# bitlayer-org/tap-stark

Measured on AMD Instinct MI355X. Metric: trace cells/sec (proofs/sec alongside), 2^20x64 BabyBear trace, higher is better.
Workload: dtype u32

## Files before the change

tap-stark_amd/csrc/ntt_lde.hip:

```cpp
#include <stdlib.h>

#include <optional>
#include <type_traits>

#include "ntt_rounds.hpp"

namespace ts {

template <int LM, bool SKIP_R16 = false>
__global__ void __launch_bounds__(chunk_threads(LM))
k_intt_contig(uint32_t* __restrict__ data, uint64_t col_stride, unsigned log_n,
              const uint32_t* __restrict__ Winv, uint32_t* __restrict__ data2, uint32_t gw) {
    __shared__ uint32_t s[padded(1 << LM)];
    const uint32_t c = blockIdx.x;
    uint32_t* col = blockIdx.y < gw ? data + (uint64_t)blockIdx.y * col_stride
                                    : data2 + (uint64_t)(blockIdx.y - gw) * col_stride;
    uint32_t* g = col + ((uint64_t)c << LM);
    chunk_load<LM>(s, g);
    chunk_rounds<LM, true, SKIP_R16>(s, log_n - LM, c, Winv);
    chunk_store<LM, false>(s, g);
}

__global__ void __launch_bounds__(256)
k_transpose_bitrev_r16(const uint32_t* __restrict__ src, uint32_t* __restrict__ dst, unsigned log_n,
                       uint32_t w, uint64_t dst_col_stride, uint32_t src_width,
                       const uint32_t* __restrict__ Winv) {
    __shared__ uint32_t tile[64][65];
    const uint32_t p0 = blockIdx.x << 6;
    const uint32_t c0 = blockIdx.y * 64;
    const uint32_t tx = threadIdx.x & 63, ty = threadIdx.x >> 6;
    const uint32_t rb = bitrev32(p0, log_n);
    const uint64_t row_step = (uint64_t)src_width << (log_n - 6);
    uint32_t v[16];
    if (c0 + tx < w) {
        const uint32_t* sp = src + (uint64_t)rb * src_width + c0 + tx;
#pragma unroll
        for (int q = 0; q < 16; q++) v[q] = sp[(uint64_t)(__brev(16 * ty + (uint32_t)q) >> 26) * row_step];
    } else {
#pragma unroll
        for (int q = 0; q < 16; q++) v[q] = 0;
    }
    radix_butterflies<4, true, false>(v, log_n - 4, 0, 0, (p0 >> 4) + ty, Winv);
#pragma unroll
    for (int q = 0; q < 16; q++) tile[16 * ty + q][tx] = v[q];
    __syncthreads();
    uint32_t t[16];
#pragma unroll
    for (int k = 0; k < 16; k++) t[k] = tile[tx][ty + 4 * k];
    uint32_t* dp = dst + (uint64_t)(c0 + ty) * dst_col_stride + p0 + tx;
#pragma unroll
    for (int k = 0; k < 16; k++)
        if (c0 + ty + 4 * k < w) dp[(uint64_t)(4 * k) * dst_col_stride] = t[k];
}

template <int LM, int CPW>
__device__ __forceinline__ void lde_fwd_contig_block(uint32_t* __restrict__ out, uint64_t out_col_stride, unsigned log_n,
                                                     const uint32_t* __restrict__ W, const uint32_t beta) {
    __shared__ uint32_t s[padded(1 << LM)];
    constexpr int NT = chunk_threads(LM);
    constexpr int NV = (1 << LM) / 4 / NT;
    uint32_t* col = out + (uint64_t)blockIdx.y * out_col_stride + ((uint64_t)beta << log_n);
    if constexpr (CPW == 1) {
        const uint32_t c = blockIdx.x;
        uint32_t* o = col + ((uint64_t)c << LM);
        chunk_load<LM>(s, o);
        chunk_rounds<LM, false>(s, log_n - LM, c, W);
        chunk_store<LM, true>(s, o);
    } else {
        const uint32_t c0 = blockIdx.x * CPW;
        uint4 v[NV];
        {
            const uint4* g4 = reinterpret_cast<const uint4*>(col + ((uint64_t)c0 << LM));
#pragma unroll
            for (int k = 0; k < NV; k++) v[k] = g4[threadIdx.x + (uint32_t)k * NT];
        }
#pragma unroll 1
        for (int i = 0; i < CPW; i++) {
            const uint32_t c = c0 + i;
#pragma unroll
            for (int k = 0; k < NV; k++) {
                const uint32_t i4 = threadIdx.x + (uint32_t)k * NT;
                const uint32_t a = 4 * i4 + (i4 >> 3);
                s[a] = v[k].x;
                s[a + 1] = v[k].y;
                s[a + 2] = v[k].z;
                s[a + 3] = v[k].w;
            }
            __syncthreads();
            if (i + 1 < CPW) {
                const uint4* g4 = reinterpret_cast<const uint4*>(col + ((uint64_t)(c + 1) << LM));
#pragma unroll
                for (int k = 0; k < NV; k++) v[k] = g4[threadIdx.x + (uint32_t)k * NT];
            }
            chunk_rounds<LM, false>(s, log_n - LM, c, W);
            chunk_store<LM, true>(s, col + ((uint64_t)c << LM));
            __syncthreads();
        }
    }
}

template <int LM, int CPW = 1>
__global__ void __launch_bounds__(chunk_threads(LM), CPW > 1 ? 4 : 1)
k_lde_fwd_contig(uint32_t* __restrict__ out, uint64_t out_col_stride, unsigned log_n,
                 const uint32_t* __restrict__ W) {
    lde_fwd_contig_block<LM, CPW>(out, out_col_stride, log_n, W, blockIdx.z);
}

template <int LM, int CPW = 1>
__global__ void __launch_bounds__(chunk_threads(LM), CPW > 1 ? 4 : 1)
k_lde_fwd_contig_own(uint32_t* __restrict__ out, uint64_t out_col_stride, unsigned log_n,
                     const uint32_t* __restrict__ W, uint32_t gw, uint32_t own_a, uint32_t own_b) {
    const uint32_t own = blockIdx.y < gw ? own_a : own_b;
    lde_fwd_contig_block<LM, CPW>(out, out_col_stride, log_n, W, blockIdx.z + (blockIdx.z >= own ? 1u : 0u));
}

template <int PLAN, int TILE = TILE_ELEMS, int NTM = NT_MID, int LM = LOG_M, bool OWN = false>
__global__ void __launch_bounds__(NTM)
k_lde_mid(const uint32_t* __restrict__ evals, uint64_t in_col_stride, uint32_t* __restrict__ out,
          uint64_t out_col_stride, unsigned log_n, unsigned log_len, unsigned log_T,
          unsigned row_shift, unsigned beta0, unsigned n_cosets, const uint32_t* __restrict__ W,
          const uint32_t* __restrict__ Winv, const uint32_t* __restrict__ scale_a,
          const uint32_t* __restrict__ evals2, const uint32_t* __restrict__ scale_b, uint32_t gw,
          uint32_t own_a, uint32_t own_b) {
    __shared__ uint32_t s[padded(TILE)];
    constexpr int PER_THREAD = TILE / NTM;
    if (PLAN == 1) {
        log_len = 8;
        log_T = 5;
    }
    const bool remap = PLAN == 0 && log_T < 5 && gridDim.x >= 8;
    uint32_t bx = remap ? (blockIdx.x & 7) * (gridDim.x >> 3) + (blockIdx.x >> 3) : blockIdx.x;
    uint32_t col_id = blockIdx.y;
    if constexpr (PLAN == 1) {
        const uint32_t ncols = gridDim.x >> (LM - 5);
        bx = (blockIdx.x & 31) + 32 * (blockIdx.x / (32 * ncols));
        col_id = (blockIdx.x >> 5) % ncols;
    }
    const uint32_t j2_0 = bx << log_T;
    const uint32_t* g = (col_id < gw ? evals + (uint64_t)col_id * in_col_stride
                                     : evals2 + (uint64_t)(col_id - gw) * in_col_stride) + j2_0;
    const uint32_t* __restrict__ scale = col_id < gw ? scale_a : scale_b;
    const uint32_t own = OWN ? (col_id < gw ? own_a : own_b) : 0xffffffffu;
    const uint32_t total = 1u << (log_len + log_T);
    const uint32_t tmask = (1u << log_T) - 1;
    if constexpr (PLAN == 1) {
        uint32_t t[PER_THREAD];
#pragma unroll
        for (int k = 0; k < PER_THREAD; k++) {
            const uint32_t i = threadIdx.x + (uint32_t)k * NTM;
            t[k] = g[((uint64_t)(i >> log_T) << row_shift) + (i & tmask)];
        }
#pragma unroll
        for (int k = 0; k < PER_THREAD; k++) s[pad(threadIdx.x + (uint32_t)k * NTM)] = t[k];
    } else {
        for (uint32_t i = threadIdx.x; i < total; i += NTM)
            s[pad(i)] = g[((uint64_t)(i >> log_T) << row_shift) + (i & tmask)];
    }
    __syncthreads();
    if (PLAN == 1) {
        radix_round<4, true, 5, NTM>(s, 13, 4, 0, 0, Winv);
    } else {
        tile_inverse_rt<NTM>(s, log_len, log_T, 0, 0, Winv);
    }
    uint32_t coef[PER_THREAD];
#pragma unroll
    for (int k = 0; k < PER_THREAD; k++) {
        const uint32_t i = threadIdx.x + (uint32_t)k * NTM;
        coef[k] = i < total ? s[pad(i)] : 0u;
    }
    constexpr int GP = PER_THREAD / 16;
    if constexpr (PLAN == 1) {
#pragma unroll
        for (int j = 0; j < GP; j++) {
            uint32_t v[16];
#pragma unroll
            for (int q = 0; q < 16; q++) v[q] = coef[j + GP * q];
            radix_butterflies<4, true, true>(v, 0, 0, 0, 0, Winv);
#pragma unroll
            for (int q = 0; q < 16; q++) coef[j + GP * q] = v[q];
        }
    }
    constexpr bool PREFETCH = PLAN == 1;
    uint32_t scv[PREFETCH ? 16 : 1];
    const uint32_t* scp = nullptr;
    if constexpr (PREFETCH) {
        const uint32_t i0 = threadIdx.x;
        scp = scale + ((uint64_t)(i0 >> 5) << LM) + (i0 & 31) + j2_0;
        const uint32_t first = OWN && own == 0 ? 1u : 0u;
#pragma unroll
        for (int q = 0; q < 16; q++)
            scv[q] = (scp + ((uint64_t)(beta0 + first) << log_n))[(uint64_t)q * (NTM >> 5) << LM];
    }
    for (uint32_t bl = 0; bl < n_cosets; bl++) {
        if (OWN && bl == own) continue;
        const uint32_t beta = beta0 + bl;
        const uint32_t* sc = scale + ((uint64_t)beta << log_n);
        __syncthreads();
        if constexpr (PLAN == 1) {
#pragma unroll
            for (int j = 0; j < GP; j++) {
                uint32_t v[16];
#pragma unroll
                for (int q = 0; q < 16; q++) v[q] = mont_mul_lazy(coef[j + GP * q], scv[q]);
                const uint32_t nb = OWN && bl + 1 == own ? bl + 2 : bl + 1;
                if (nb < n_cosets) {
                    const uint32_t* nx = scp + ((uint64_t)(beta0 + nb) << log_n);
#pragma unroll
                    for (int q = 0; q < 16; q++) scv[q] = nx[(uint64_t)q * (NTM >> 5) << LM];
                }
                radix_butterflies<4, false, true>(v, 0, 0, 0, 0, W);
#pragma unroll
                for (int q = 0; q < 16; q++) s[pad(threadIdx.x + (uint32_t)(j + GP * q) * NTM)] = v[q];
            }
            __syncthreads();
            uint32_t* og = out + (uint64_t)col_id * out_col_stride + ((uint64_t)bl << log_n) + j2_0;
            radix_round<4, false, 5, NTM>(s, 13, 4, 0, 0, W);
            uint32_t t[PER_THREAD];
#pragma unroll
            for (int k = 0; k < PER_THREAD; k++) t[k] = s[pad(threadIdx.x + (uint32_t)k * NTM)];
            uint32_t* ot = og + ((uint64_t)(threadIdx.x >> 5) << LM) + (threadIdx.x & 31);
#pragma unroll
            for (int k = 0; k < PER_THREAD; k++) ot[(uint64_t)k * (NTM >> 5) << LM] = t[k];
            continue;
        } else {
#pragma unroll
            for (int k = 0; k < PER_THREAD; k++) {
                const uint32_t i = threadIdx.x + (uint32_t)k * NTM;
                if (i < total) {
                    const uint32_t kk = ((i >> log_T) << row_shift) + (i & tmask) + j2_0;
                    s[pad(i)] = mont_mul_lazy(coef[k], sc[kk]);
                }
            }
            __syncthreads();
            tile_forward_rt<NTM>(s, log_len, log_T, 0, 0, W);
        }
        uint32_t* o = out + (uint64_t)col_id * out_col_stride + ((uint64_t)bl << log_n) + j2_0;
        if (row_shift != 0) {
            for (uint32_t i = threadIdx.x; i < total; i += NTM)
                o[((uint64_t)(i >> log_T) << row_shift) + (i & tmask)] = s[pad(i)];
        } else {
            for (uint32_t i = threadIdx.x; i < total; i += NTM)
                o[((uint64_t)(i >> log_T) << row_shift) + (i & tmask)] = red2p(s[pad(i)]);
        }
    }
}

template <bool VEC>
__global__ void __launch_bounds__(256)
k_lde_own_copy(const uint32_t* __restrict__ evals, uint64_t in_col_stride, uint32_t* __restrict__ out,
               uint64_t out_col_stride, unsigned log_n, const uint32_t* __restrict__ evals2, uint32_t gw,
               uint32_t own_a, uint32_t own_b) {
    const uint32_t col = blockIdx.y;
    const uint32_t* src = col < gw ? evals + (uint64_t)col * in_col_stride
                                   : evals2 + (uint64_t)(col - gw) * in_col_stride;
    uint32_t* dst = out + (uint64_t)col * out_col_stride + ((uint64_t)(col < gw ? own_a : own_b) << log_n);
    if constexpr (VEC) {
        const uint4* s4 = reinterpret_cast<const uint4*>(src) + (uint64_t)blockIdx.x * 1024 + threadIdx.x;
        uint4* d4 = reinterpret_cast<uint4*>(dst) + (uint64_t)blockIdx.x * 1024 + threadIdx.x;
        uint4 v[4];
#pragma unroll
        for (int k = 0; k < 4; k++) v[k] = s4[256 * k];
#pragma unroll
        for (int k = 0; k < 4; k++) d4[256 * k] = v[k];
    } else {
        const uint64_t i = (uint64_t)blockIdx.x * 256 + threadIdx.x;
        if (i < (1ull << log_n)) dst[i] = src[i];
    }
}

constexpr const char* INTT_NAME[3] = {"k_intt_contig<12>", "k_intt_contig<13>", "k_intt_contig<14>"};
constexpr const char* INTT_R16_NAME[3] = {"(k_intt_contig<12, true>)", "(k_intt_contig<13, true>)",
                                          "(k_intt_contig<14, true>)"};
constexpr const char* FWD_NAME[3] = {"k_lde_fwd_contig<12>", "k_lde_fwd_contig<13>", "(k_lde_fwd_contig<14, 4>)"};

template <class F>
static void with_chunk_log(unsigned LM, F&& f) {
    if (LM == 12) f(std::integral_constant<int, 12>{});
    else if (LM == 13) f(std::integral_constant<int, 13>{});
    else f(std::integral_constant<int, 14>{});
}

bool launch_transpose_bitrev_r16(Context& ctx, const uint32_t* src, uint32_t* dst, unsigned log_n, uint32_t w,
                                 uint64_t dst_col_stride, uint32_t src_width) {
    if (w == 0 || !ntt_plan(log_n).fused_first_round) return false;
    ctx.ensure_twiddles(log_n);
    TS_LAUNCH(ctx, k_transpose_bitrev_r16, dim3(1u << (log_n - 6), (w + 63) / 64), dim3(256), 0, src, dst, log_n, w,
              dst_col_stride, src_width ? src_width : w, (const uint32_t*)ctx.d_twiddle_inv);
    TS_HIP(hipGetLastError());
    return true;
}

void launch_contig_inverse(Context& ctx, const NttPlan& p, uint32_t* data, uint64_t col_stride, uint32_t ncols,
                           bool first_round_done, uint32_t* data2, uint32_t gw) {
    const uint32_t* Winv = ctx.d_twiddle_inv;
    with_chunk_log(p.LM, [&](auto lm) {
        constexpr int LM = decltype(lm)::value;
        const dim3 g(p.chunks, ncols), b(chunk_threads(LM));
        if (first_round_done)
            TS_LAUNCH_NAMED(ctx, INTT_R16_NAME[LM - 12], (k_intt_contig<LM, true>), g, b, 0, data, col_stride, p.log_n,
                            Winv, data2, gw);
        else
            TS_LAUNCH_NAMED(ctx, INTT_NAME[LM - 12], k_intt_contig<LM>, g, b, 0, data, col_stride, p.log_n, Winv, data2,
                            gw);
    });
}

static void launch_lde_mid(Context& ctx, const NttPlan& p, const uint32_t* evals, uint64_t in_col_stride,
                           uint32_t* out, uint64_t out_col_stride, uint32_t ncols, uint32_t beta0, uint32_t n_beta,
                           const uint32_t* scale, const uint32_t* evals2, const uint32_t* scale2, uint32_t gw,
                           uint32_t own_a, uint32_t own_b) {
    const uint32_t *W = ctx.d_twiddle_fwd, *Winv = ctx.d_twiddle_inv;
    const dim3 grid(p.tiles, ncols), b(NT_MID);
    const dim3 grid1(p.tiles * ncols);
#define TS_MID_ARGS \
    evals, in_col_stride, out, out_col_stride, p.log_n, p.log_len, p.log_T, p.row_shift, beta0, n_beta, W, Winv, scale, \
        evals2, scale2, gw, own_a, own_b
    if (own_a != LDE_NO_OWN && p.mid == NttMid::FIXED256 && p.LM == 12)
        TS_LAUNCH_NAMED(ctx, "k_lde_mid<1>", (k_lde_mid<1, TILE_ELEMS, NT_MID, 12, true>), grid1, b, 0, TS_MID_ARGS);
    else if (own_a != LDE_NO_OWN && p.mid == NttMid::FIXED256 && p.LM == 13)
        TS_LAUNCH_NAMED(ctx, "(k_lde_mid<1, 8192, 512, 13>)", (k_lde_mid<1, 8192, 512, 13, true>), grid1, b, 0,
                        TS_MID_ARGS);
    else if (own_a != LDE_NO_OWN && p.mid == NttMid::FIXED256)
        TS_LAUNCH_NAMED(ctx, "(k_lde_mid<1, 8192, 512, 14>)", (k_lde_mid<1, 8192, 512, 14, true>), grid1, b, 0,
                        TS_MID_ARGS);
    else if (own_a != LDE_NO_OWN)
        TS_LAUNCH_NAMED(ctx, "k_lde_mid<0>", (k_lde_mid<0, TILE_ELEMS, NT_MID, LOG_M, true>), grid, b, 0, TS_MID_ARGS);
    else if (p.mid == NttMid::TILE16384)
        TS_LAUNCH_NAMED(ctx, "(k_lde_mid<0, 16384>)", (k_lde_mid<0, 16384>), grid, b, 0, TS_MID_ARGS);
    else if (p.mid == NttMid::FIXED256 && p.LM == 12)
        TS_LAUNCH_NAMED(ctx, "k_lde_mid<1>", k_lde_mid<1>, grid1, b, 0, TS_MID_ARGS);
    else if (p.mid == NttMid::FIXED256 && p.LM == 13)
        TS_LAUNCH_NAMED(ctx, "(k_lde_mid<1, 8192, 512, 13>)", (k_lde_mid<1, 8192, 512, 13>), grid1, b, 0, TS_MID_ARGS);
    else if (p.mid == NttMid::FIXED256)
        TS_LAUNCH_NAMED(ctx, "(k_lde_mid<1, 8192, 512, 14>)", (k_lde_mid<1, 8192, 512, 14>), grid1, b, 0, TS_MID_ARGS);
    else
        TS_LAUNCH_NAMED(ctx, "k_lde_mid<0>", k_lde_mid<0>, grid, b, 0, TS_MID_ARGS);
#undef TS_MID_ARGS
}

void launch_contig_forward(Context& ctx, const NttPlan& p, uint32_t* data, uint64_t col_stride, uint32_t ncols,
                           uint32_t n_blocks, uint32_t gw, uint32_t own_a, uint32_t own_b) {
    const uint32_t* W = ctx.d_twiddle_fwd;
    with_chunk_log(p.LM, [&](auto lm) {
        constexpr int LM = decltype(lm)::value;
        constexpr int CPW = LM == 14 ? 4 : 1;
        if (own_a != LDE_NO_OWN)
            TS_LAUNCH_NAMED(ctx, FWD_NAME[LM - 12], (k_lde_fwd_contig_own<LM, CPW>),
                            dim3(p.chunks / CPW, ncols, n_blocks - 1), dim3(chunk_threads(LM)), 0, data, col_stride,
                            p.log_n, W, gw, own_a, own_b);
        else
            TS_LAUNCH_NAMED(ctx, FWD_NAME[LM - 12], (k_lde_fwd_contig<LM, CPW>), dim3(p.chunks / CPW, ncols, n_blocks),
                            dim3(chunk_threads(LM)), 0, data, col_stride, p.log_n, W);
    });
}

int lde_own_coset_used(unsigned log_n, unsigned log_blowup, uint32_t shift) {
    if (const char* e = getenv("TS_LDE_OWN_COSET"); e && *e && atoi(e) == 0) return -1;
    if (log_blowup == 0 || log_n + log_blowup > 27 || ntt_plan(log_n).mid == NttMid::TILE16384) return -1;
    return lde_own_coset(log_n, log_blowup, shift);
}

void coset_lde(Context& ctx, uint32_t* evals, uint64_t in_col_stride, uint32_t ncols, unsigned log_n,
               unsigned log_blowup, uint32_t shift, uint32_t* out, uint64_t out_col_stride,
               uint32_t beta0, uint32_t n_beta, bool first_round_done, uint32_t* evals2, uint32_t shift2,
               uint32_t gw, bool stage_timers) {
    if (ncols == 0) return;
    TS_REQUIRE(evals2 == nullptr || (gw >= 1 && gw < ncols && shift2 != 0), TS_ERR_INVALID,
               "coset_lde: second matrix needs its first column and its shift");
    if (evals2 == nullptr) gw = 0xffffffffu;
    TS_REQUIRE(log_n + log_blowup <= 27, TS_ERR_INVALID, "coset_lde: log_n + log_blowup > 27");
    const NttPlan p = ntt_plan(log_n);
    ntt_require_shape(p, ncols, in_col_stride, out_col_stride, true);
    TS_REQUIRE(!first_round_done || p.fused_first_round, TS_ERR_INVARIANT,
               "coset_lde: no contiguous inverse pass at this size");
    ctx.ensure_twiddles(log_n == 0 ? 1 : log_n);

    const uint32_t n_cosets = 1u << log_blowup;
    if (n_beta == 0) n_beta = n_cosets - beta0;
    TS_REQUIRE(beta0 < n_cosets && n_beta <= n_cosets - beta0, TS_ERR_INVALID, "coset_lde: coset range");
    const uint32_t* scale = coset_scale_table(ctx, log_n, log_blowup, shift);
    const uint32_t* scale2 = evals2 ? coset_scale_table(ctx, log_n, log_blowup, shift2) : nullptr;

    uint32_t own_a = LDE_NO_OWN, own_b = LDE_NO_OWN;
    if (beta0 == 0 && n_beta == n_cosets && !first_round_done && ctx.lde_pass_mask == 7u) {
        const int a = lde_own_coset_used(log_n, log_blowup, shift);
        const int b = evals2 ? lde_own_coset_used(log_n, log_blowup, shift2) : a;
        if (a >= 0 && b >= 0) {
            own_a = (uint32_t)a;
            own_b = (uint32_t)b;
            const uint64_t n = 1ull << log_n;
            if (p.two_pass)
                TS_LAUNCH_NAMED(ctx, "k_lde_own_copy", k_lde_own_copy<true>, dim3((unsigned)(n >> 12), ncols), dim3(256), 0,
                                (const uint32_t*)evals, in_col_stride, out, out_col_stride, log_n,
                                (const uint32_t*)evals2, gw, own_a, own_b);
            else
                TS_LAUNCH_NAMED(ctx, "k_lde_own_copy", k_lde_own_copy<false>, dim3((unsigned)((n + 255) / 256), ncols),
                                dim3(256), 0, (const uint32_t*)evals, in_col_stride, out, out_col_stride, log_n,
                                (const uint32_t*)evals2, gw, own_a, own_b);
        }
    }

    if (!p.two_pass) {
        launch_lde_mid(ctx, p, evals, in_col_stride, out, out_col_stride, ncols, beta0, n_beta, scale, evals2, scale2,
                       gw, own_a, own_b);
    } else {
        if (ctx.lde_pass_mask & 1u) {
            std::optional<StageTimer> t;
            if (stage_timers) t.emplace(&ctx, "lde: inverse NTT, contiguous stages");
            launch_contig_inverse(ctx, p, evals, in_col_stride, ncols, first_round_done, evals2, gw);
        }
        std::optional<StageTimer> t_rest;
        if (stage_timers) t_rest.emplace(&ctx, "lde: strided pass + forward NTT of the owned cosets");
        if (ctx.lde_pass_mask & 2u)
            launch_lde_mid(ctx, p, evals, in_col_stride, out, out_col_stride, ncols, beta0, n_beta, scale, evals2,
                           scale2, gw, own_a, own_b);
        if (ctx.lde_pass_mask & 4u) launch_contig_forward(ctx, p, out, out_col_stride, ncols, n_beta, gw, own_a, own_b);
    }
    TS_HIP(hipGetLastError());
}

}
```

tap-stark_amd/csrc/open.hip:

```cpp
#include "kernels.hpp"

namespace ts {

__device__ __forceinline__ uint32_t root_bitrev(const uint32_t* __restrict__ W, unsigned L, uint64_t r) {
    if (L == 0) return R_MOD_P;
    uint32_t w = W[((uint64_t)1 << (L - 1)) + (r >> 1)];
    return (r & 1) ? neg(w) : w;
}

constexpr int BW_ROWS = 4;

__global__ void __launch_bounds__(256)
k_bary_weights(unsigned log_n, const uint32_t* __restrict__ W, uint32_t gen_mont, Ef z0, Ef z1,
               uint32_t n_points, Ef* __restrict__ out) {
    const uint64_t n = 1ull << log_n;
    const uint64_t t0 = ((uint64_t)blockIdx.x * blockDim.x + threadIdx.x) * BW_ROWS;
    if (t0 >= n) return;
    Ef num[2 * BW_ROWS];
    uint32_t nrm[2 * BW_ROWS], pre[2 * BW_ROWS], xs[BW_ROWS];
    uint32_t run = R_MOD_P;
#pragma unroll
    for (int k = 0; k < BW_ROWS; k++) {
        const bool ok = t0 + k < n;
        uint32_t x = ok ? mont_mul(gen_mont, root_bitrev(W, log_n, t0 + k)) : R_MOD_P;
        xs[k] = x;
#pragma unroll
        for (int p = 0; p < 2; p++) {
            const Ef z = p == 0 ? z0 : z1;
            Ef u = Ef{{sub(z.c[0], x), z.c[1], z.c[2], z.c[3]}};
            if (p < (int)n_points && ok) {
                ef_inv_parts(u, num[2 * k + p], nrm[2 * k + p]);
            } else {
                num[2 * k + p] = ef_zero();
                nrm[2 * k + p] = R_MOD_P;
            }
            pre[2 * k + p] = run;
            run = mont_mul(run, nrm[2 * k + p]);
        }
    }
    uint32_t inv = mont_inv(run);
#pragma unroll
    for (int j = 2 * BW_ROWS - 1; j >= 0; j--) {
        uint32_t ninv = mont_mul(inv, pre[j]);
        inv = mont_mul(inv, nrm[j]);
        const int k = j >> 1, p = j & 1;
        if (p < (int)n_points && t0 + k < n)
            out[(uint64_t)p * n + t0 + k] = ef_mul_base(num[j], mont_mul(ninv, xs[k]));
    }
}

void launch_bary_weights(Context& ctx, unsigned log_n, const Ef* points_mont, uint32_t n_points,
                         Ef* out, uint32_t coset_gen) {
    TS_REQUIRE(n_points >= 1 && n_points <= 2, TS_ERR_INVALID, "bary_weights: 1 or 2 points");
    ctx.ensure_twiddles(log_n == 0 ? 1 : log_n);
    const uint64_t threads = (((uint64_t)1 << log_n) + BW_ROWS - 1) / BW_ROWS;
    Ef z0 = points_mont[0], z1 = n_points > 1 ? points_mont[1] : points_mont[0];
    TS_LAUNCH(ctx, k_bary_weights, dim3((unsigned)((threads + 255) / 256)), dim3(256), 0, log_n,
              ctx.d_twiddle_fwd, to_mont(coset_gen ? coset_gen : GENERATOR), z0, z1, n_points, out);
    TS_HIP(hipGetLastError());
}

template <int NP, int COLS>
__global__ void __launch_bounds__(256)
k_bary_dots(const uint32_t* __restrict__ m, uint64_t col_stride, uint32_t width, unsigned log_n,
            const Ef* __restrict__ weights, uint32_t* __restrict__ partial, uint32_t rows_per_block) {
    constexpr int RS = 64 / COLS;
    constexpr int TR = 16 * 4 * RS;
    constexpr int PER_THREAD = COLS * TR / 256;
    __shared__ uint32_t tile[16 * 257];
    __shared__ uint32_t wts[TR][NP * 4];
    __shared__ uint32_t red[4 * RS][COLS][NP * 4];
    const uint64_t n = 1ull << log_n;
    const uint32_t c0 = blockIdx.y * COLS;
    const uint32_t lane = threadIdx.x & 63, wv = threadIdx.x >> 6;
    const uint32_t cl = lane % COLS, rs = lane / COLS;
    const uint32_t sub = wv * RS + rs;
    const uint64_t row_begin = (uint64_t)blockIdx.x * rows_per_block;
    const uint64_t row_end = row_begin + rows_per_block < n ? row_begin + rows_per_block : n;
    uint64_t acc[NP * 4];
#pragma unroll
    for (int j = 0; j < NP * 4; j++) acc[j] = 0;
    for (uint64_t row0 = row_begin; row0 < row_end; row0 += TR) {
        uint32_t v[PER_THREAD];
#pragma unroll
        for (int k = 0; k < PER_THREAD; k++) {
            const uint32_t e = threadIdx.x + (uint32_t)k * 256;
            const uint32_t c = c0 + e / TR;
            const uint64_t t = row0 + e % TR;
            v[k] = (c < width && t < row_end) ? m[(uint64_t)c * col_stride + t] : 0u;
        }
        for (uint32_t e = threadIdx.x; e < (uint32_t)(TR * NP); e += 256) {
            const uint32_t p = e / TR, tt = e % TR;
            const uint64_t t = row0 + tt;
            Ef w = ef_zero();
            if (t < row_end) w = weights[(uint64_t)p * n + t];
            wts[tt][p * 4 + 0] = w.c[0];
            wts[tt][p * 4 + 1] = w.c[1];
            wts[tt][p * 4 + 2] = w.c[2];
            wts[tt][p * 4 + 3] = w.c[3];
        }
#pragma unroll
        for (int k = 0; k < PER_THREAD; k++) {
            const uint32_t e = threadIdx.x + (uint32_t)k * 256;
            const uint32_t t = e % TR;
            tile[(t & 15) * 257 + (t >> 4) * COLS + e / TR] = v[k];
        }
        __syncthreads();
#pragma unroll
        for (int rr = 0; rr < 16; rr++) {
            const uint32_t tt = sub * 16 + rr;
            const uint32_t x = tile[rr * 257 + sub * COLS + cl];
#pragma unroll
            for (int j = 0; j < NP * 4; j++) acc[j] = lazy_mac(acc[j], x, wts[tt][j]);
            if (rr & 1) {
#pragma unroll
                for (int j = 0; j < NP * 4; j++) acc[j] = lazy_fix(acc[j]);
            }
        }
        __syncthreads();
    }
#pragma unroll
    for (int j = 0; j < NP * 4; j++) red[sub][cl][j] = lazy_finish(acc[j]);
    __syncthreads();
    for (uint32_t idx = threadIdx.x; idx < (uint32_t)(COLS * NP * 4); idx += 256) {
        const uint32_t c = idx / (NP * 4), j = idx % (NP * 4);
        uint32_t sum = 0;
#pragma unroll
        for (int q = 0; q < 4 * RS; q++) sum = add(sum, red[q][c][j]);
        if (c0 + c < width)
            partial[((uint64_t)blockIdx.x * width + c0 + c) * (NP * 4) + j] = sum;
    }
}

struct BaryFinishJob {
    const uint32_t* partial;
    uint32_t* out;
    uint32_t n_blocks, n_words;
};
__device__ __forceinline__ void bary_finish_group(const uint32_t* __restrict__ partial, uint32_t* __restrict__ out,
                                                  uint32_t n_blocks, uint32_t n_words, uint32_t group) {
    __shared__ uint32_t red[4][4];
    const uint32_t j = group * 4 + (threadIdx.x & 3);
    uint32_t v = 0;
    if (j < n_words) {
        uint32_t b = threadIdx.x >> 2;
        for (; b + 7 * 64 < n_blocks; b += 8 * 64) {
            uint32_t x[8];
#pragma unroll
            for (int k = 0; k < 8; k++) x[k] = partial[(uint64_t)(b + 64 * k) * n_words + j];
#pragma unroll
            for (int k = 0; k < 8; k++) v = add(v, x[k]);
        }
        for (; b < n_blocks; b += 64) v = add(v, partial[(uint64_t)b * n_words + j]);
    }
#pragma unroll
    for (int off = 32; off >= 4; off >>= 1) v = add(v, __shfl_down(v, off, 64));
    const uint32_t lane = threadIdx.x & 63, wv = threadIdx.x >> 6;
    if (lane < 4) red[wv][lane] = v;
    __syncthreads();
    if (threadIdx.x < 4 && j < n_words)
        out[j] = add(add(red[0][threadIdx.x], red[1][threadIdx.x]),
                     add(red[2][threadIdx.x], red[3][threadIdx.x]));
}
__global__ void __launch_bounds__(256)
k_bary_finish(BaryFinishJob j0, BaryFinishJob j1, uint32_t g0) {
    const bool first = blockIdx.x < g0;
    bary_finish_group(first ? j0.partial : j1.partial, first ? j0.out : j1.out, first ? j0.n_blocks : j1.n_blocks,
                      first ? j0.n_words : j1.n_words, first ? blockIdx.x : blockIdx.x - g0);
}
__global__ void __launch_bounds__(256)
k_bary_finish3(BaryFinishJob j0, BaryFinishJob j1, BaryFinishJob j2, uint32_t g0, uint32_t g1) {
    const BaryFinishJob j = blockIdx.x < g0 ? j0 : blockIdx.x < g0 + g1 ? j1 : j2;
    bary_finish_group(j.partial, j.out, j.n_blocks, j.n_words,
                      blockIdx.x < g0 ? blockIdx.x : blockIdx.x < g0 + g1 ? blockIdx.x - g0 : blockIdx.x - g0 - g1);
}

__global__ void __launch_bounds__(256)
k_bary_finish4(BaryFinishJob j0, BaryFinishJob j1, BaryFinishJob j2, BaryFinishJob j3, uint32_t g0, uint32_t g1,
               uint32_t g2) {
    const uint32_t b = blockIdx.x;
    const BaryFinishJob j = b < g0 ? j0 : b < g0 + g1 ? j1 : b < g0 + g1 + g2 ? j2 : j3;
    bary_finish_group(j.partial, j.out, j.n_blocks, j.n_words,
                      b < g0 ? b : b < g0 + g1 ? b - g0 : b < g0 + g1 + g2 ? b - g0 - g1 : b - g0 - g1 - g2);
}

void launch_bary_finish(Context& ctx, BaryPending& pend) {
    if (pend.n == 0) return;
    BaryFinishJob j[4] = {{nullptr, nullptr, 0, 0}, {nullptr, nullptr, 0, 0}, {nullptr, nullptr, 0, 0},
                          {nullptr, nullptr, 0, 0}};
    uint32_t g[4] = {0, 0, 0, 0};
    for (uint32_t i = 0; i < pend.n; i++) {
        j[i] = BaryFinishJob{pend.partial[i].p, pend.out[i], pend.n_blocks[i], pend.n_words[i]};
        g[i] = (pend.n_words[i] + 3) / 4;
    }
    if (pend.n == 4)
        TS_LAUNCH(ctx, k_bary_finish4, dim3(g[0] + g[1] + g[2] + g[3]), dim3(256), 0, j[0], j[1], j[2], j[3], g[0], g[1],
                  g[2]);
    else if (pend.n == 3)
        TS_LAUNCH(ctx, k_bary_finish3, dim3(g[0] + g[1] + g[2]), dim3(256), 0, j[0], j[1], j[2], g[0], g[1]);
    else
        TS_LAUNCH(ctx, k_bary_finish, dim3(g[0] + g[1]), dim3(256), 0, j[0], j[1], g[0]);
    TS_HIP(hipGetLastError());
    for (uint32_t i = 0; i < pend.n; i++) pend.partial[i].reset();
    pend.n = 0;
}

void launch_bary_dots(Context& ctx, const ColMat& m, unsigned log_n, const Ef* weights,
                      uint32_t n_points, Ef* out, BaryPending* pending) {
    const uint64_t n = 1ull << log_n;
    const bool narrow = m.width <= 8;
    const uint32_t tr = narrow ? 512 : 64;
    uint32_t n_blocks = (uint32_t)((n + tr - 1) / tr);
    if (n_blocks > 2048) n_blocks = 2048;
    uint32_t rows_per_block = (uint32_t)(((n + n_blocks - 1) / n_blocks + tr - 1) / tr * tr);
    n_blocks = (uint32_t)((n + rows_per_block - 1) / rows_per_block);
    const uint32_t n_words = m.width * n_points * 4;
    DevBuf<uint32_t> partial(&ctx, (size_t)n_blocks * n_words);
    const uint32_t* md = m.d;
    if (narrow) {
        dim3 grid(n_blocks, (m.width + 7) / 8);
        if (n_points == 2)
            TS_LAUNCH(ctx, (k_bary_dots<2, 8>), grid, dim3(256), 0, md, m.col_stride, m.width, log_n,
                      weights, partial.p, rows_per_block);
        else
            TS_LAUNCH(ctx, (k_bary_dots<1, 8>), grid, dim3(256), 0, md, m.col_stride, m.width, log_n,
                      weights, partial.p, rows_per_block);
    } else {
        dim3 grid(n_blocks, (m.width + 63) / 64);
        if (n_points == 2)
            TS_LAUNCH(ctx, (k_bary_dots<2, 64>), grid, dim3(256), 0, md, m.col_stride, m.width, log_n,
                      weights, partial.p, rows_per_block);
        else
            TS_LAUNCH(ctx, (k_bary_dots<1, 64>), grid, dim3(256), 0, md, m.col_stride, m.width, log_n,
                      weights, partial.p, rows_per_block);
    }
    TS_HIP(hipGetLastError());
    BaryPending own;
    BaryPending& pend = pending ? *pending : own;
    if (pend.n == pend.capacity) launch_bary_finish(ctx, pend);
    pend.partial[pend.n] = std::move(partial);
    pend.out[pend.n] = reinterpret_cast<uint32_t*>(out);
    pend.n_blocks[pend.n] = n_blocks;
    pend.n_words[pend.n] = n_words;
    pend.n++;
    if (!pending) launch_bary_finish(ctx, pend);
}

__device__ __forceinline__ void row_dot_acc(uint64_t (&acc)[4], const uint32_t* __restrict__ m,
                                            uint64_t col_stride, uint32_t width, uint64_t X,
                                            const uint32_t* __restrict__ weights) {
    uint64_t a0 = acc[0], a1 = acc[1], a2 = acc[2], a3 = acc[3];
    constexpr int B = 8;
    const uint32_t* col = m + X;
    uint32_t i = 0;
    for (; i + B <= width; i += B) {
        uint32_t v[B];
#pragma unroll
        for (int k = 0; k < B; k++) v[k] = col[(uint64_t)(i + k) * col_stride];
#pragma unroll
        for (int k = 0; k < B; k++) {
            const uint32_t* ap = weights + 4 * (i + k);
            a0 = lazy_mac(a0, v[k], ap[0]);
            a1 = lazy_mac(a1, v[k], ap[1]);
            a2 = lazy_mac(a2, v[k], ap[2]);
            a3 = lazy_mac(a3, v[k], ap[3]);
            if (k & 1) {
                a0 = lazy_fix(a0);
                a1 = lazy_fix(a1);
                a2 = lazy_fix(a2);
                a3 = lazy_fix(a3);
            }
        }
    }
    if (i < width) {
        uint32_t v[B];
#pragma unroll
        for (int k = 0; k < B; k++) v[k] = i + k < width ? col[(uint64_t)(i + k) * col_stride] : 0u;
#pragma unroll
        for (int k = 0; k < B; k++) {
            if (i + k < width) {
                const uint32_t* ap = weights + 4 * (i + k);
                a0 = lazy_mac(a0, v[k], ap[0]);
                a1 = lazy_mac(a1, v[k], ap[1]);
                a2 = lazy_mac(a2, v[k], ap[2]);
                a3 = lazy_mac(a3, v[k], ap[3]);
            }
            if (k & 1) {
                a0 = lazy_fix(a0);
                a1 = lazy_fix(a1);
                a2 = lazy_fix(a2);
                a3 = lazy_fix(a3);
            }
        }
    }
    acc[0] = a0; acc[1] = a1; acc[2] = a2; acc[3] = a3;
}
__device__ __forceinline__ Ef row_dot_alpha(const uint32_t* __restrict__ m, uint64_t col_stride,
                                            uint32_t width, uint64_t X,
                                            const uint32_t* __restrict__ alpha_pows) {
    uint64_t acc[4] = {0, 0, 0, 0};
    row_dot_acc(acc, m, col_stride, width, X, alpha_pows);
    return Ef{{lazy_finish(acc[0]), lazy_finish(acc[1]), lazy_finish(acc[2]), lazy_finish(acc[3])}};
}

template <int NP>
__device__ __forceinline__ void inv_denoms(uint32_t x_mont, const Ef* z_mont, Ef* out) {
    Ef num[NP];
    uint32_t nrm[NP];
#pragma unroll
    for (int p = 0; p < NP; p++) {
        const Ef z = z_mont[p];
        Ef u = Ef{{sub(x_mont, z.c[0]), neg(z.c[1]), neg(z.c[2]), neg(z.c[3])}};
        ef_inv_parts(u, num[p], nrm[p]);
    }
    if (NP == 2) {
        uint32_t inv = mont_inv(mont_mul(nrm[0], nrm[NP - 1]));
        out[0] = ef_mul_base(num[0], mont_mul(inv, nrm[NP - 1]));
        out[NP - 1] = ef_mul_base(num[NP - 1], mont_mul(inv, nrm[0]));
    } else {
        out[0] = ef_mul_base(num[0], mont_inv(nrm[0]));
    }
}

template <int NP>
__global__ void __launch_bounds__(256)
k_reduce(const uint32_t* __restrict__ m, uint64_t col_stride, uint32_t width, unsigned log_h,
         const uint32_t* __restrict__ W, uint32_t gen_mont, const uint32_t* __restrict__ alpha_pows,
         ReduceArgs args, Ef* __restrict__ ro) {
    const uint64_t h = 1ull << log_h;
    const uint64_t X = (uint64_t)blockIdx.x * blockDim.x + threadIdx.x;
    if (X >= h) return;
    const Ef S = row_dot_alpha(m, col_stride, width, X, alpha_pows);
    const uint32_t x = mont_mul(gen_mont, root_bitrev(W, log_h, X));
    Ef inv_d[NP];
    inv_denoms<NP>(x, args.z_mont, inv_d);
    Ef acc = args.accumulate ? ro[X] : ef_zero();
#pragma unroll
    for (int p = 0; p < NP; p++) {
        Ef t = ef_mul(ef_sub(S, args.rys[p]), args.off_mont[p]);
        acc = ef_add(acc, ef_mul(t, inv_d[p]));
    }
    ro[X] = acc;
}

void launch_reduce(Context& ctx, const ColMat& m, unsigned log_h, const uint32_t* d_alpha_pows_mont,
                   const ReduceArgs& args, Ef* ro) {
    TS_REQUIRE(args.n_points >= 1 && args.n_points <= 2, TS_ERR_INVALID, "reduce: 1 or 2 points");
    ctx.ensure_twiddles(log_h == 0 ? 1 : log_h);
    const uint64_t h = 1ull << log_h;
    dim3 grid((unsigned)((h + 255) / 256));
    if (args.n_points == 2)
        TS_LAUNCH(ctx, k_reduce<2>, grid, dim3(256), 0, (const uint32_t*)m.d, m.col_stride, m.width,
                  log_h, (const uint32_t*)ctx.d_twiddle_fwd, to_mont(GENERATOR), d_alpha_pows_mont, args,
                  ro);
    else
        TS_LAUNCH(ctx, k_reduce<1>, grid, dim3(256), 0, (const uint32_t*)m.d, m.col_stride, m.width,
                  log_h, (const uint32_t*)ctx.d_twiddle_fwd, to_mont(GENERATOR), d_alpha_pows_mont, args,
                  ro);
    TS_HIP(hipGetLastError());
}

__global__ void __launch_bounds__(256)
k_reduce_fused(const uint32_t* __restrict__ trace, uint64_t trace_stride, uint32_t width,
               unsigned log_h, const uint32_t* __restrict__ W, uint32_t gen_mont,
               const uint32_t* __restrict__ alpha_pows, FusedReduceArgs a, Ef* __restrict__ ro) {
    const uint64_t X = (uint64_t)blockIdx.x * blockDim.x + threadIdx.x;
    if (X >= a.rows) return;
    const Ef St = row_dot_alpha(trace, trace_stride, width, X, alpha_pows);
    const uint32_t x = mont_mul(gen_mont, root_bitrev(W, log_h, a.row0 + X));
    Ef inv_d[2];
    inv_denoms<2>(x, a.z_mont, inv_d);
    uint64_t acc[4] = {0, 0, 0, 0};
    uint32_t c = 0;
    for (; c + 2 <= a.n_chunks; c += 2) {
        uint32_t v[8];
#pragma unroll
        for (int k = 0; k < 8; k++) v[k] = a.chunk[c + (k >> 2)][(uint64_t)(k & 3) * a.chunk_stride + X];
        const uint32_t* ap = a.chunk_w + 16 * c;
#pragma unroll
        for (int k = 0; k < 8; k++) {
#pragma unroll
            for (int j = 0; j < 4; j++) acc[j] = lazy_mac(acc[j], v[k], ap[4 * k + j]);
            if (k & 1) {
#pragma unroll
                for (int j = 0; j < 4; j++) acc[j] = lazy_fix(acc[j]);
            }
        }
    }
    for (; c < a.n_chunks; c++) row_dot_acc(acc, a.chunk[c], a.chunk_stride, 4, X, a.chunk_w + 16 * c);
    const Ef D{{lazy_finish(acc[0]), lazy_finish(acc[1]), lazy_finish(acc[2]), lazy_finish(acc[3])}};
    const Ef g0 = ef_sub(ef_add(ef_mul(St, a.off_t[0]), D), a.k0);
    const Ef g1 = ef_sub(ef_mul(St, a.off_t[1]), a.k1);
    const Ef r = ef_add(ef_mul(g0, inv_d[0]), ef_mul(g1, inv_d[1]));
    *reinterpret_cast<uint4*>(ro + X) = make_uint4(r.c[0], r.c[1], r.c[2], r.c[3]);
}

struct PrepReduceArgs {
    const uint32_t* prep;
    uint64_t stride;
    uint32_t width;
    Ef off_p[2];
};
__global__ void __launch_bounds__(256)
k_reduce_fused_pre(const uint32_t* __restrict__ trace, uint64_t trace_stride, uint32_t width,
               unsigned log_h, const uint32_t* __restrict__ W, uint32_t gen_mont,
               const uint32_t* __restrict__ alpha_pows, FusedReduceArgs a, PrepReduceArgs pa,
               Ef* __restrict__ ro) {
    const uint64_t X = (uint64_t)blockIdx.x * blockDim.x + threadIdx.x;
    if (X >= a.rows) return;
    const Ef St = row_dot_alpha(trace, trace_stride, width, X, alpha_pows);
    const uint32_t x = mont_mul(gen_mont, root_bitrev(W, log_h, a.row0 + X));
    Ef inv_d[2];
    inv_denoms<2>(x, a.z_mont, inv_d);
    uint64_t acc[4] = {0, 0, 0, 0};
    uint32_t c = 0;
    for (; c + 2 <= a.n_chunks; c += 2) {
        uint32_t v[8];
#pragma unroll
        for (int k = 0; k < 8; k++) v[k] = a.chunk[c + (k >> 2)][(uint64_t)(k & 3) * a.chunk_stride + X];
        const uint32_t* ap = a.chunk_w + 16 * c;
#pragma unroll
        for (int k = 0; k < 8; k++) {
#pragma unroll
            for (int j = 0; j < 4; j++) acc[j] = lazy_mac(acc[j], v[k], ap[4 * k + j]);
            if (k & 1) {
#pragma unroll
                for (int j = 0; j < 4; j++) acc[j] = lazy_fix(acc[j]);
            }
        }
    }
    for (; c < a.n_chunks; c++) row_dot_acc(acc, a.chunk[c], a.chunk_stride, 4, X, a.chunk_w + 16 * c);
    const Ef D{{lazy_finish(acc[0]), lazy_finish(acc[1]), lazy_finish(acc[2]), lazy_finish(acc[3])}};
    const Ef Sp = row_dot_alpha(pa.prep, pa.stride, pa.width, X, alpha_pows);
    const Ef g0 = ef_sub(ef_add(ef_add(ef_mul(St, a.off_t[0]), ef_mul(Sp, pa.off_p[0])), D), a.k0);
    const Ef g1 = ef_sub(ef_add(ef_mul(St, a.off_t[1]), ef_mul(Sp, pa.off_p[1])), a.k1);
    const Ef r = ef_add(ef_mul(g0, inv_d[0]), ef_mul(g1, inv_d[1]));
    *reinterpret_cast<uint4*>(ro + X) = make_uint4(r.c[0], r.c[1], r.c[2], r.c[3]);
}

struct PrepAuxReduceArgs {
    const uint32_t* prep;
    const uint32_t* aux;
    uint64_t prep_stride, aux_stride;
    uint32_t prep_width, aux_width;
    Ef off_p[2];
    Ef off_a[2];
};
__global__ void __launch_bounds__(256)
k_reduce_fused_pre_aux(const uint32_t* __restrict__ trace, uint64_t trace_stride, uint32_t width,
                       unsigned log_h, const uint32_t* __restrict__ W, uint32_t gen_mont,
                       const uint32_t* __restrict__ alpha_pows, FusedReduceArgs a, PrepAuxReduceArgs pa,
                       Ef* __restrict__ ro) {
    const uint64_t X = (uint64_t)blockIdx.x * blockDim.x + threadIdx.x;
    if (X >= a.rows) return;
    const Ef St = row_dot_alpha(trace, trace_stride, width, X, alpha_pows);
    const uint32_t x = mont_mul(gen_mont, root_bitrev(W, log_h, a.row0 + X));
    Ef inv_d[2];
    inv_denoms<2>(x, a.z_mont, inv_d);
    uint64_t acc[4] = {0, 0, 0, 0};
    uint32_t c = 0;
    for (; c + 2 <= a.n_chunks; c += 2) {
        uint32_t v[8];
#pragma unroll
        for (int k = 0; k < 8; k++) v[k] = a.chunk[c + (k >> 2)][(uint64_t)(k & 3) * a.chunk_stride + X];
        const uint32_t* ap = a.chunk_w + 16 * c;
#pragma unroll
        for (int k = 0; k < 8; k++) {
#pragma unroll
            for (int j = 0; j < 4; j++) acc[j] = lazy_mac(acc[j], v[k], ap[4 * k + j]);
            if (k & 1) {
#pragma unroll
                for (int j = 0; j < 4; j++) acc[j] = lazy_fix(acc[j]);
            }
        }
    }
    for (; c < a.n_chunks; c++) row_dot_acc(acc, a.chunk[c], a.chunk_stride, 4, X, a.chunk_w + 16 * c);
    const Ef D{{lazy_finish(acc[0]), lazy_finish(acc[1]), lazy_finish(acc[2]), lazy_finish(acc[3])}};
    const Ef Sp = row_dot_alpha(pa.prep, pa.prep_stride, pa.prep_width, X, alpha_pows);
    const Ef Sa = row_dot_alpha(pa.aux, pa.aux_stride, pa.aux_width, X, alpha_pows);
    const Ef g0 = ef_sub(ef_add(ef_add(ef_add(ef_mul(St, a.off_t[0]), ef_mul(Sp, pa.off_p[0])), ef_mul(Sa, pa.off_a[0])), D),
                         a.k0);
    const Ef g1 = ef_sub(ef_add(ef_add(ef_mul(St, a.off_t[1]), ef_mul(Sp, pa.off_p[1])), ef_mul(Sa, pa.off_a[1])), a.k1);
    const Ef r = ef_add(ef_mul(g0, inv_d[0]), ef_mul(g1, inv_d[1]));
    *reinterpret_cast<uint4*>(ro + X) = make_uint4(r.c[0], r.c[1], r.c[2], r.c[3]);
}

void launch_reduce_fused(Context& ctx, const ColMat& trace, unsigned log_h,
                         const uint32_t* d_alpha_pows_mont, const FusedReduceArgs& args, Ef* ro,
                         const ColMat* prep, const Ef* prep_off_mont, const ColMat* aux, const Ef* aux_off_mont) {
    TS_REQUIRE(args.n_chunks <= (uint32_t)MAX_QUOTIENT_CHUNKS, TS_ERR_INVALID, "reduce_fused: too many chunks");
    ctx.ensure_twiddles(log_h == 0 ? 1 : log_h);
    FusedReduceArgs a = args;
    if (a.rows == 0) {
        a.row0 = 0;
        a.rows = 1ull << log_h;
    }
    TS_REQUIRE(a.row0 + a.rows <= (1ull << log_h), TS_ERR_INVALID, "reduce_fused: row range");
    TS_REQUIRE(!aux || prep, TS_ERR_INVARIANT, "reduce_fused: a third matrix without a second");
    if (aux) {
        for (const ColMat* m : {prep, aux})
            TS_REQUIRE(m->d && a.row0 == 0 && m->height == a.rows && m->col_stride >= a.rows, TS_ERR_INVALID,
                       "reduce_fused: preprocessed or aux matrix shape");
        TS_REQUIRE(prep_off_mont && aux_off_mont, TS_ERR_INVALID, "reduce_fused: missing offsets");
        const PrepAuxReduceArgs pa{prep->d, aux->d, prep->col_stride, aux->col_stride, prep->width, aux->width,
                                   {prep_off_mont[0], prep_off_mont[1]}, {aux_off_mont[0], aux_off_mont[1]}};
        TS_LAUNCH(ctx, k_reduce_fused_pre_aux, dim3((unsigned)((a.rows + 255) / 256)), dim3(256), 0,
                  (const uint32_t*)trace.d, trace.col_stride, trace.width, log_h,
                  (const uint32_t*)ctx.d_twiddle_fwd, to_mont(GENERATOR), d_alpha_pows_mont, a, pa, ro);
        TS_HIP(hipGetLastError());
        return;
    }
    if (prep) {
        TS_REQUIRE(prep_off_mont && prep->d && a.row0 == 0 && prep->height == a.rows && prep->col_stride >= a.rows,
                   TS_ERR_INVALID, "reduce_fused: preprocessed matrix shape");
        const PrepReduceArgs pa{prep->d, prep->col_stride, prep->width, {prep_off_mont[0], prep_off_mont[1]}};
        TS_LAUNCH(ctx, k_reduce_fused_pre, dim3((unsigned)((a.rows + 255) / 256)), dim3(256), 0,
                  (const uint32_t*)trace.d, trace.col_stride, trace.width, log_h,
                  (const uint32_t*)ctx.d_twiddle_fwd, to_mont(GENERATOR), d_alpha_pows_mont, a, pa, ro);
        TS_HIP(hipGetLastError());
        return;
    }
    TS_LAUNCH(ctx, k_reduce_fused, dim3((unsigned)((a.rows + 255) / 256)), dim3(256), 0,
              (const uint32_t*)trace.d, trace.col_stride, trace.width, log_h,
              (const uint32_t*)ctx.d_twiddle_fwd, to_mont(GENERATOR), d_alpha_pows_mont, a, ro);
    TS_HIP(hipGetLastError());
}

__device__ __forceinline__ Ef chunk_dot(const FusedReduceArgs& a, uint64_t X) {
    uint64_t acc[4] = {0, 0, 0, 0};
    uint32_t c = 0;
    for (; c + 2 <= a.n_chunks; c += 2) {
        uint32_t v[8];
#pragma unroll
        for (int k = 0; k < 8; k++) v[k] = a.chunk[c + (k >> 2)][(uint64_t)(k & 3) * a.chunk_stride + X];
        const uint32_t* ap = a.chunk_w + 16 * c;
#pragma unroll
        for (int k = 0; k < 8; k++) {
#pragma unroll
            for (int j = 0; j < 4; j++) acc[j] = lazy_mac(acc[j], v[k], ap[4 * k + j]);
            if (k & 1) {
#pragma unroll
                for (int j = 0; j < 4; j++) acc[j] = lazy_fix(acc[j]);
            }
        }
    }
    for (; c < a.n_chunks; c++) row_dot_acc(acc, a.chunk[c], a.chunk_stride, 4, X, a.chunk_w + 16 * c);
    return Ef{{lazy_finish(acc[0]), lazy_finish(acc[1]), lazy_finish(acc[2]), lazy_finish(acc[3])}};
}

__global__ void __launch_bounds__(256)
k_reduce_low(const uint32_t* __restrict__ trace, uint64_t trace_stride, uint32_t width, unsigned log_n,
             const uint32_t* __restrict__ Winv, uint32_t gen_inv_mont, const uint32_t* __restrict__ alpha_pows,
             FusedReduceArgs a, const Ef* __restrict__ weights, uint32_t* __restrict__ out) {
    const uint64_t n = 1ull << log_n;
    const uint64_t t = (uint64_t)blockIdx.x * blockDim.x + threadIdx.x;
    if (t >= n) return;
    const Ef St = row_dot_alpha(trace, trace_stride, width, t, alpha_pows);
    const Ef D = chunk_dot(a, t);
    const uint32_t nxi = neg(mont_mul(gen_inv_mont, root_bitrev(Winv, log_n, t)));
    const Ef inv_d0 = ef_mul_base(weights[t], nxi), inv_d1 = ef_mul_base(weights[n + t], nxi);
    const Ef g0 = ef_sub(ef_add(ef_mul(St, a.off_t[0]), D), a.k0);
    const Ef g1 = ef_sub(ef_mul(St, a.off_t[1]), a.k1);
    const Ef r = ef_add(ef_mul(g0, inv_d0), ef_mul(g1, inv_d1));
#pragma unroll
    for (int k = 0; k < 4; k++) out[(uint64_t)k * n + t] = r.c[k];
}

void launch_reduce_low(Context& ctx, const ColMat& trace, unsigned log_n, const uint32_t* d_alpha_pows_mont,
                       const FusedReduceArgs& args, const Ef* weights, uint32_t* out) {
    TS_REQUIRE(args.n_chunks <= (uint32_t)MAX_QUOTIENT_CHUNKS, TS_ERR_INVALID, "reduce_low: too many chunks");
    const uint64_t n = 1ull << log_n;
    TS_REQUIRE(args.row0 == 0 && trace.height >= n && trace.col_stride >= n && args.chunk_stride >= n, TS_ERR_INVALID,
               "reduce_low: the matrices must start with the low coset");
    ctx.ensure_twiddles(log_n == 0 ? 1 : log_n);
    TS_LAUNCH(ctx, k_reduce_low, dim3((unsigned)((n + 255) / 256)), dim3(256), 0, (const uint32_t*)trace.d,
              trace.col_stride, trace.width, log_n, (const uint32_t*)ctx.d_twiddle_inv,
              to_mont(inv_canon(GENERATOR)), d_alpha_pows_mont, args, weights, out);
    TS_HIP(hipGetLastError());
}

__global__ void __launch_bounds__(256)
k_ef_interleave(const uint32_t* __restrict__ cols, uint64_t col_stride, uint64_t rows, Ef* __restrict__ out) {
    const uint64_t X = (uint64_t)blockIdx.x * blockDim.x + threadIdx.x;
    if (X >= rows) return;
    *reinterpret_cast<uint4*>(out + X) = make_uint4(cols[X], cols[col_stride + X], cols[2 * col_stride + X],
                                                    cols[3 * col_stride + X]);
}

void launch_ef_interleave(Context& ctx, const uint32_t* cols, uint64_t col_stride, uint64_t rows, Ef* out) {
    TS_REQUIRE(col_stride >= rows, TS_ERR_INVALID, "ef_interleave: column stride below the row count");
    TS_LAUNCH(ctx, k_ef_interleave, dim3((unsigned)((rows + 255) / 256)), dim3(256), 0, cols, col_stride, rows, out);
    TS_HIP(hipGetLastError());
}

}
```

Baseline: 26.01 billion.

## Use wave-uniform base pointers with 32-bit offsets in LDE mid and barycentric dots

Adds helpers that force a base pointer into scalar registers with readfirstlane and address global memory through a 32-bit per-lane byte offset, so loads and stores can use the SGPR-base plus VGPR-offset form instead of 64-bit per-lane address arithmetic. The fixed LDE mid kernel gets a 2D grid that removes the division and modulo in block index decoding, and its coset loop now double-buffers the scale prefetch in two register arrays. The barycentric dot kernel precomputes per-column uniform pointers and clamps row offsets. The code relies on byte offsets fitting in 32 bits and on a new invariant checked at launch.

```diff
diff --git a/tap-stark_amd/csrc/ntt_lde.hip b/tap-stark_amd/csrc/ntt_lde.hip
--- a/tap-stark_amd/csrc/ntt_lde.hip
+++ b/tap-stark_amd/csrc/ntt_lde.hip
@@ -4,6 +4,7 @@
 #include <type_traits>
 
 #include "ntt_rounds.hpp"
+#include "uaddr.hpp"
 
 namespace ts {
 
@@ -132,9 +133,8 @@
     uint32_t bx = remap ? (blockIdx.x & 7) * (gridDim.x >> 3) + (blockIdx.x >> 3) : blockIdx.x;
     uint32_t col_id = blockIdx.y;
     if constexpr (PLAN == 1) {
-        const uint32_t ncols = gridDim.x >> (LM - 5);
-        bx = (blockIdx.x & 31) + 32 * (blockIdx.x / (32 * ncols));
-        col_id = (blockIdx.x >> 5) % ncols;
+        bx = (blockIdx.x & 31) + 32 * blockIdx.y;
+        col_id = blockIdx.x >> 5;
     }
     const uint32_t j2_0 = bx << log_T;
     const uint32_t* g = (col_id < gw ? evals + (uint64_t)col_id * in_col_stride
@@ -143,13 +143,12 @@
     const uint32_t own = OWN ? (col_id < gw ? own_a : own_b) : 0xffffffffu;
     const uint32_t total = 1u << (log_len + log_T);
     const uint32_t tmask = (1u << log_T) - 1;
+    const uint32_t lane_off = (((threadIdx.x >> 5) << LM) | (threadIdx.x & 31)) * 4u;
+    constexpr uint64_t row_step = (uint64_t)(NTM >> 5) << LM;
     if constexpr (PLAN == 1) {
         uint32_t t[PER_THREAD];
 #pragma unroll
-        for (int k = 0; k < PER_THREAD; k++) {
-            const uint32_t i = threadIdx.x + (uint32_t)k * NTM;
-            t[k] = g[((uint64_t)(i >> log_T) << row_shift) + (i & tmask)];
-        }
+        for (int k = 0; k < PER_THREAD; k++) t[k] = ld_ub(row_base(g, k * row_step), lane_off);
 #pragma unroll
         for (int k = 0; k < PER_THREAD; k++) s[pad(threadIdx.x + (uint32_t)k * NTM)] = t[k];
     } else {
@@ -180,49 +179,50 @@
             for (int q = 0; q < 16; q++) coef[j + GP * q] = v[q];
         }
     }
-    constexpr bool PREFETCH = PLAN == 1;
-    uint32_t scv[PREFETCH ? 16 : 1];
-    const uint32_t* scp = nullptr;
-    if constexpr (PREFETCH) {
-        const uint32_t i0 = threadIdx.x;
-        scp = scale + ((uint64_t)(i0 >> 5) << LM) + (i0 & 31) + j2_0;
-        const uint32_t first = OWN && own == 0 ? 1u : 0u;
-#pragma unroll
-        for (int q = 0; q < 16; q++)
-            scv[q] = (scp + ((uint64_t)(beta0 + first) << log_n))[(uint64_t)q * (NTM >> 5) << LM];
-    }
-    for (uint32_t bl = 0; bl < n_cosets; bl++) {
-        if (OWN && bl == own) continue;
-        const uint32_t beta = beta0 + bl;
-        const uint32_t* sc = scale + ((uint64_t)beta << log_n);
-        __syncthreads();
-        if constexpr (PLAN == 1) {
-#pragma unroll
-            for (int j = 0; j < GP; j++) {
-                uint32_t v[16];
-#pragma unroll
-                for (int q = 0; q < 16; q++) v[q] = mont_mul_lazy(coef[j + GP * q], scv[q]);
-                const uint32_t nb = OWN && bl + 1 == own ? bl + 2 : bl + 1;
-                if (nb < n_cosets) {
-                    const uint32_t* nx = scp + ((uint64_t)(beta0 + nb) << log_n);
-#pragma unroll
-                    for (int q = 0; q < 16; q++) scv[q] = nx[(uint64_t)q * (NTM >> 5) << LM];
-                }
-                radix_butterflies<4, false, true>(v, 0, 0, 0, 0, W);
-#pragma unroll
-                for (int q = 0; q < 16; q++) s[pad(threadIdx.x + (uint32_t)(j + GP * q) * NTM)] = v[q];
-            }
-            __syncthreads();
-            uint32_t* og = out + (uint64_t)col_id * out_col_stride + ((uint64_t)bl << log_n) + j2_0;
+    if constexpr (PLAN == 1) {
+        static_assert(GP == 1, "the prefetch below replaces the scale set of the only group");
+        const uint32_t* scp = scale + j2_0;
+        uint32_t* og = out + (uint64_t)col_id * out_col_stride + j2_0;
+        auto prefetch = [&](uint32_t (&sc)[16], uint32_t bl) {
+            const uint32_t so = lane_off + ((beta0 + bl) << log_n) * 4u;
+#pragma unroll
+            for (int q = 0; q < 16; q++) sc[q] = ld_ub(row_base(scp, q * row_step), so);
+        };
+        auto next_coset = [&](uint32_t bl) { return OWN && bl + 1 == own ? bl + 2 : bl + 1; };
+        auto coset = [&](uint32_t bl, uint32_t nb, const uint32_t (&sc)[16], uint32_t (&nx)[16]) {
+            __syncthreads();
+            uint32_t v[16];
+#pragma unroll
+            for (int q = 0; q < 16; q++) v[q] = mont_mul_lazy(coef[q], sc[q]);
+            if (nb < n_cosets) prefetch(nx, nb);
+            radix_butterflies<4, false, true>(v, 0, 0, 0, 0, W);
+#pragma unroll
+            for (int q = 0; q < 16; q++) s[pad(threadIdx.x + (uint32_t)q * NTM)] = v[q];
+            __syncthreads();
             radix_round<4, false, 5, NTM>(s, 13, 4, 0, 0, W);
             uint32_t t[PER_THREAD];
 #pragma unroll
             for (int k = 0; k < PER_THREAD; k++) t[k] = s[pad(threadIdx.x + (uint32_t)k * NTM)];
-            uint32_t* ot = og + ((uint64_t)(threadIdx.x >> 5) << LM) + (threadIdx.x & 31);
-#pragma unroll
-            for (int k = 0; k < PER_THREAD; k++) ot[(uint64_t)k * (NTM >> 5) << LM] = t[k];
-            continue;
-        } else {
+            const uint32_t oo = lane_off + (bl << log_n) * 4u;
+#pragma unroll
+            for (int k = 0; k < PER_THREAD; k++) st_ub(row_base(og, k * row_step), oo, t[k]);
+        };
+        uint32_t sca[16], scb[16];
+        uint32_t bl = OWN && own == 0 ? 1u : 0u;
+        prefetch(sca, bl);
+        while (bl < n_cosets) {
+            uint32_t nb = next_coset(bl);
+            coset(bl, nb, sca, scb);
+            if (nb >= n_cosets) break;
+            bl = next_coset(nb);
+            coset(nb, bl, scb, sca);
+        }
+    } else {
+        for (uint32_t bl = 0; bl < n_cosets; bl++) {
+            if (OWN && bl == own) continue;
+            const uint32_t beta = beta0 + bl;
+            const uint32_t* sc = scale + ((uint64_t)beta << log_n);
+            __syncthreads();
 #pragma unroll
             for (int k = 0; k < PER_THREAD; k++) {
                 const uint32_t i = threadIdx.x + (uint32_t)k * NTM;
@@ -233,14 +233,14 @@
             }
             __syncthreads();
             tile_forward_rt<NTM>(s, log_len, log_T, 0, 0, W);
-        }
-        uint32_t* o = out + (uint64_t)col_id * out_col_stride + ((uint64_t)bl << log_n) + j2_0;
-        if (row_shift != 0) {
-            for (uint32_t i = threadIdx.x; i < total; i += NTM)
-                o[((uint64_t)(i >> log_T) << row_shift) + (i & tmask)] = s[pad(i)];
-        } else {
-            for (uint32_t i = threadIdx.x; i < total; i += NTM)
-                o[((uint64_t)(i >> log_T) << row_shift) + (i & tmask)] = red2p(s[pad(i)]);
+            uint32_t* o = out + (uint64_t)col_id * out_col_stride + ((uint64_t)bl << log_n) + j2_0;
+            if (row_shift != 0) {
+                for (uint32_t i = threadIdx.x; i < total; i += NTM)
+                    o[((uint64_t)(i >> log_T) << row_shift) + (i & tmask)] = s[pad(i)];
+            } else {
+                for (uint32_t i = threadIdx.x; i < total; i += NTM)
+                    o[((uint64_t)(i >> log_T) << row_shift) + (i & tmask)] = red2p(s[pad(i)]);
+            }
         }
     }
 }
@@ -311,7 +311,9 @@
                            uint32_t own_a, uint32_t own_b) {
     const uint32_t *W = ctx.d_twiddle_fwd, *Winv = ctx.d_twiddle_inv;
     const dim3 grid(p.tiles, ncols), b(NT_MID);
-    const dim3 grid1(p.tiles * ncols);
+    const dim3 grid1(32 * ncols, p.tiles / 32);
+    TS_REQUIRE(p.mid != NttMid::FIXED256 || (p.row_shift == p.LM && p.tiles % 32 == 0), TS_ERR_INVARIANT,
+               "lde_mid: the fixed plan has rows 2^LM apart and a multiple of 32 tiles");
 #define TS_MID_ARGS \
     evals, in_col_stride, out, out_col_stride, p.log_n, p.log_len, p.log_T, p.row_shift, beta0, n_beta, W, Winv, scale, \
         evals2, scale2, gw, own_a, own_b
diff --git a/tap-stark_amd/csrc/open.hip b/tap-stark_amd/csrc/open.hip
--- a/tap-stark_amd/csrc/open.hip
+++ b/tap-stark_amd/csrc/open.hip
@@ -1,4 +1,5 @@
 #include "kernels.hpp"
+#include "uaddr.hpp"
 
 namespace ts {
 
@@ -80,14 +81,30 @@
     uint64_t acc[NP * 4];
 #pragma unroll
     for (int j = 0; j < NP * 4; j++) acc[j] = 0;
-    for (uint64_t row0 = row_begin; row0 < row_end; row0 += TR) {
+    const uint32_t n_rows = row_begin < row_end ? (uint32_t)(row_end - row_begin) : 0u;
+    const uint32_t wave_u = __builtin_amdgcn_readfirstlane(wv);
+    const uint32_t* colb[PER_THREAD];
+    {
+        const uint32_t first = c0 + (TR == 64 ? wave_u : 0u);
+        const uint32_t* col = m + (uint64_t)(first < width ? first : c0) * col_stride + row_begin;
+#pragma unroll
+        for (int k = 0; k < PER_THREAD; k++) {
+            const uint32_t dc = k == 0 ? 0u : TR == 64 ? 4u : (uint32_t)(~k & 1);
+            const uint32_t c = c0 + (TR == 64 ? wave_u + 4u * (uint32_t)k : (uint32_t)k * 256u / TR);
+            if (dc != 0 && c < width) col += (uint64_t)dc * col_stride;
+            colb[k] = uniform_ptr(col);
+        }
+    }
+    for (uint32_t r0 = 0; r0 < n_rows; r0 += TR) {
+        const uint64_t row0 = row_begin + r0;
         uint32_t v[PER_THREAD];
 #pragma unroll
         for (int k = 0; k < PER_THREAD; k++) {
             const uint32_t e = threadIdx.x + (uint32_t)k * 256;
             const uint32_t c = c0 + e / TR;
-            const uint64_t t = row0 + e % TR;
-            v[k] = (c < width && t < row_end) ? m[(uint64_t)c * col_stride + t] : 0u;
+            const uint32_t t = r0 + e % TR;
+            const uint32_t x = ld_ub(colb[k], (t < n_rows ? t : n_rows - 1) * 4u);
+            v[k] = (c < width && t < n_rows) ? x : 0u;
         }
         for (uint32_t e = threadIdx.x; e < (uint32_t)(TR * NP); e += 256) {
             const uint32_t p = e / TR, tt = e % TR;
diff --git a/tap-stark_amd/csrc/uaddr.hpp b/tap-stark_amd/csrc/uaddr.hpp
--- /dev/null
+++ b/tap-stark_amd/csrc/uaddr.hpp
@@ -0,0 +1,32 @@
+#pragma once
+#include <stdint.h>
+
+#include <hip/hip_runtime.h>
+
+namespace ts {
+
+template <class T>
+__device__ __forceinline__ T* uniform_ptr(T* p) {
+    const uint64_t a = reinterpret_cast<uint64_t>(p);
+    const uint32_t lo = __builtin_amdgcn_readfirstlane((uint32_t)a);
+    const uint32_t hi = __builtin_amdgcn_readfirstlane((uint32_t)(a >> 32));
+    using G = __attribute__((address_space(1))) T;
+    return (T*)reinterpret_cast<G*>(((uint64_t)hi << 32) | lo);
+}
+
+template <class T>
+__device__ __forceinline__ T* row_base(T* base, uint64_t elems) {
+    return uniform_ptr(base + elems);
+}
+
+template <class T = uint32_t>
+__device__ __forceinline__ T ld_ub(const T* __restrict__ base, uint32_t byte_off) {
+    return *reinterpret_cast<const T*>(reinterpret_cast<const char*>(base) + byte_off);
+}
+
+template <class T = uint32_t>
+__device__ __forceinline__ void st_ub(T* __restrict__ base, uint32_t byte_off, T v) {
+    *reinterpret_cast<T*>(reinterpret_cast<char*>(base) + byte_off) = v;
+}
+
+}
```

Result: no change. 25.99 billion (-0.1%).
